# 2alaaa/distributed-llm-scheduler

Hardware: AMD Instinct MI355X
Metric: DAG makespan (ms) + tasks completed under mem cap, GPT-2 DAG at 1/2/4/8 MI355X (lower is better)
Workload: dtype bf16

## Files before the change

csrc/kernels/gemm_glds_impl.h:

```cpp
#pragma once
#include <cstdlib>
#include <type_traits>
#include "common.h"
#include "kernels.h"
#include "gemm_glds_cfgs.h"

#ifndef DLS_STAMP
#define DLS_STAMP(k)
#endif

namespace {

__device__ __forceinline__ int kslice_count(int K, int kslice) { return K / kslice; }

template <int N>
__device__ __forceinline__ void wait_vm() {
  asm volatile("s_waitcnt vmcnt(%0)" ::"n"(N) : "memory");
}
template <int PW, int A>
__device__ __forceinline__ void wait_tiles(int ahead) {
  if constexpr (A == 0) {
    wait_vm<0>();
  } else {
    if (ahead >= A) wait_vm<PW * A>();
    else wait_tiles<PW, A - 1>(ahead);
  }
}
__device__ __forceinline__ void raw_barrier() { asm volatile("s_barrier" ::: "memory"); }

template <int BM_, int BN_, int WM_, int WN_, int STAGES_, int PRIO_ = 0, int BXS_ = 0, int KG_ = 1, int RING_ = 0,
          int OCC_ = 1>
struct Cfg {
  static constexpr int BM = BM_, BN = BN_, WM = WM_, WN = WN_, STAGES = STAGES_, PRIO = PRIO_, BXS = BXS_;
  static constexpr int KG = KG_, RING = RING_, OCC = OCC_;
  static constexpr int BK = 64, CH = 8;
  static constexpr int NW = WM * WN, T = 64 * NW * KG;
  static constexpr int WTM = BM / WM, WTN = BN / WN, FM = WTM / 16, FN = WTN / 16;
  static constexpr bool HALF_FRAGS = FM + FN > 12;
  static constexpr int ROWS = BM + BN, INSTR = ROWS / 8, PW = (INSTR + NW - 1) / NW;
  static constexpr int SUB = ROWS * CH;
  static constexpr int STAGE = SUB * KG;
  static constexpr int SA = STAGES, SB = STAGES + BXS;
  static constexpr int PWA = (BM / 8 + NW - 1) / NW, PWB = (BN / 8 + NW - 1) / NW;
  static constexpr bool EVEN = INSTR % NW == 0, EVEN_A = (BM / 8) % NW == 0, EVEN_B = (BN / 8) % NW == 0;
  static constexpr int A_STAGE = BM * CH, B_STAGE = BN * CH;
  static constexpr int LDS_UNITS = BXS ? SA * A_STAGE + SB * B_STAGE : STAGES * STAGE;
  static_assert(BM % 8 == 0 && BN % 8 == 0, "DMA pieces are 8 rows");
  static_assert(FM >= 1 && FN >= 1, "wave tile too small");
  static_assert(PW * (STAGES - 2) <= 63, "vmcnt range");
  static_assert(!BXS || (SA - 2) * PWA + (SA - 1) * PWB <= 63, "vmcnt range (split rings)");
  static_assert(STAGES >= 2 && STAGES <= 8, "stages");
  static_assert(LDS_UNITS * 16 <= 163840, "LDS budget");
  static_assert(KG == 1 || (BXS == 0 && PRIO == 0), "K groups use the joint ring");
  static_assert(KG == 1 || NW * 64 * FM * FN * 16 <= LDS_UNITS * 16, "K-group reduction must fit the LDS");
  static_assert(!RING || (BM == 256 && BN == 256 && WM == 2 && WN == 4 && STAGES == 2 && KG == 1 && BXS == 0),
                "the ring main loop is written for 256x256 tiles, 8 waves as 2 x 4, 8 x 16 KiB slots");
};

template <int PWA, int PWB, int AM, int BM>
__device__ __forceinline__ void wait_ab_any(int a, int b) {
  if constexpr (AM > 0) {
    if (a < AM) {
      wait_ab_any<PWA, PWB, AM - 1, BM>(a, b);
      return;
    }
  }
  if constexpr (BM > 0) {
    if (b < BM) {
      wait_ab_any<PWA, PWB, AM, BM - 1>(a, b);
      return;
    }
  }
  wait_vm<AM * PWA + BM * PWB>();
}
template <int PWA, int PWB, int A>
__device__ __forceinline__ void wait_ab(int a, int b) {
  if constexpr (A == 0) {
    if (b >= 1) wait_vm<PWB>();
    else wait_vm<0>();
  } else {
    if (a >= A) {
      if (b > A) wait_vm<A * PWA + (A + 1) * PWB>();
      else wait_vm<A * PWA + A * PWB>();
    } else {
      wait_ab<PWA, PWB, A - 1>(a, b);
    }
  }
}

template <class C, bool SKIP = false>
__device__ __forceinline__ void mma_tile(const bf16x8* sA, const bf16x8* sB, int lane, int wm, int wn, bool ln_acc,
                                         f32x4 (&acc)[C::FM][C::FN], float (&st_s)[C::FM], float (&st_q)[C::FM],
                                         int fmv = C::FM) {
  constexpr bool HALVES = C::HALF_FRAGS;
  if constexpr (!HALVES) {
    bf16x8 af[2][C::FM], bw[2][C::FN];
#pragma unroll
    for (int kk = 0; kk < 2; ++kk) {
      const int chunk = kk * 4 + (lane >> 4);
#pragma unroll
      for (int j = 0; j < C::FN; ++j) {
        const int row = wn * C::WTN + j * 16 + (lane & 15);
        bw[kk][j] = sB[row * C::CH + (chunk ^ (row & 7))];
      }
#pragma unroll
      for (int i = 0; i < C::FM; ++i) {
        if (SKIP && i >= fmv) break;
        const int row = wm * C::WTM + i * 16 + (lane & 15);
        af[kk][i] = sA[row * C::CH + (chunk ^ (row & 7))];
      }
    }
    __builtin_amdgcn_sched_barrier(0);
#pragma unroll
    for (int kk = 0; kk < 2; ++kk) {
      if (ln_acc) {
#pragma unroll
        for (int i = 0; i < C::FM; ++i)
#pragma unroll
          for (int e = 0; e < 8; ++e) {
            const float x = bf2f(af[kk][i][e]);
            st_s[i] += x;
            st_q[i] += x * x;
          }
      }
      if constexpr (C::PRIO) __builtin_amdgcn_s_setprio(1);
#pragma unroll
      for (int i = 0; i < C::FM; ++i) {
        if (SKIP && i >= fmv) break;
#pragma unroll
        for (int j = 0; j < C::FN; ++j) acc[i][j] = mfma16x16x32(bw[kk][j], af[kk][i], acc[i][j]);
      }
      if constexpr (C::PRIO) __builtin_amdgcn_s_setprio(0);
    }
  } else {
#pragma unroll
    for (int kk = 0; kk < 2; ++kk) {
      bf16x8 af[C::FM], bw[C::FN];
      const int chunk = kk * 4 + (lane >> 4);
#pragma unroll
      for (int j = 0; j < C::FN; ++j) {
        const int row = wn * C::WTN + j * 16 + (lane & 15);
        bw[j] = sB[row * C::CH + (chunk ^ (row & 7))];
      }
#pragma unroll
      for (int i = 0; i < C::FM; ++i) {
        if (SKIP && i >= fmv) break;
        const int row = wm * C::WTM + i * 16 + (lane & 15);
        af[i] = sA[row * C::CH + (chunk ^ (row & 7))];
      }
      __builtin_amdgcn_sched_barrier(0);
      if (ln_acc) {
#pragma unroll
        for (int i = 0; i < C::FM; ++i)
#pragma unroll
          for (int e = 0; e < 8; ++e) {
            const float x = bf2f(af[i][e]);
            st_s[i] += x;
            st_q[i] += x * x;
          }
      }
      if constexpr (C::PRIO) __builtin_amdgcn_s_setprio(1);
#pragma unroll
      for (int i = 0; i < C::FM; ++i) {
        if (SKIP && i >= fmv) break;
#pragma unroll
        for (int j = 0; j < C::FN; ++j) acc[i][j] = mfma16x16x32(bw[j], af[i], acc[i][j]);
      }
      if constexpr (C::PRIO) __builtin_amdgcn_s_setprio(0);
      __builtin_amdgcn_sched_barrier(0);
    }
  }
}

template <class C, bool GATHER = false, int APOL = 0, int WPOL = 0>
__device__ __forceinline__ void mainloop_joint(bf16x8* smem, const bf16* __restrict__ A, int lda,
                                               const bf16* __restrict__ W, int ldw, int M, int N, int m0, int n0,
                                               int kbeg, int nk, int lane, int wave, int kgrp, int wm, int wn,
                                               bool ln_acc, f32x4 (&acc)[C::FM][C::FN], float (&st_s)[C::FM],
                                               float (&st_q)[C::FM], const int* __restrict__ arows) {
  const bf16* src[C::PW];
  int dst[C::PW];
#pragma unroll
  for (int j = 0; j < C::PW; ++j) {
    const int gi = C::EVEN ? wave * C::PW + j : min(wave * C::PW + j, C::INSTR * C::KG - 1);
    const int sub = gi / C::INSTR, r8 = gi % C::INSTR;
    const int row = 8 * r8 + (lane >> 3);
    const int gch = (lane & 7) ^ (row & 7);
    const int kofs = kbeg + sub * C::BK + gch * 8;
    if (row < C::BM) {
      int gm = min(m0 + row, M - 1);
      if constexpr (GATHER) gm = arows[gm];
      src[j] = A + (size_t)gm * lda + kofs;
    } else {
      const int gn = min(n0 + row - C::BM, N - 1);
      src[j] = W + (size_t)gn * ldw + kofs;
    }
    dst[j] = sub * C::SUB + r8 * 64;
  }
  bool is_a[C::PW];
#pragma unroll
  for (int j = 0; j < C::PW; ++j) {
    const int gi = C::EVEN ? wave * C::PW + j : min(wave * C::PW + j, C::INSTR * C::KG - 1);
    is_a[j] = 8 * (gi % C::INSTR) < C::BM;
  }
  auto issue = [&](int kt) {
    bf16x8* stage = smem + (kt % C::STAGES) * C::STAGE;
#pragma unroll
    for (int j = 0; j < C::PW; ++j) {
      if constexpr (APOL != 0 || WPOL != 0) {
        if (is_a[j])
          __builtin_amdgcn_global_load_lds((const void*)(src[j] + kt * (C::BK * C::KG)),
                                           (__attribute__((address_space(3))) void*)(stage + dst[j]), 16, 0, APOL);
        else
          __builtin_amdgcn_global_load_lds((const void*)(src[j] + kt * (C::BK * C::KG)),
                                           (__attribute__((address_space(3))) void*)(stage + dst[j]), 16, 0, WPOL);
        continue;
      }
      __builtin_amdgcn_global_load_lds((const void*)(src[j] + kt * (C::BK * C::KG)),
                                       (__attribute__((address_space(3))) void*)(stage + dst[j]), 16, 0, 0);
    }
  };
#pragma unroll
  for (int s = 0; s < C::STAGES - 1; ++s)
    if (s < nk) issue(s);
  for (int kt = 0; kt < nk; ++kt) {
    const int ahead = min(C::STAGES - 2, nk - 1 - kt);
    wait_tiles<C::PW, C::STAGES - 2>(ahead);
    raw_barrier();
    if (kt + C::STAGES - 1 < nk) issue(kt + C::STAGES - 1);
    const bf16x8* st = smem + (kt % C::STAGES) * C::STAGE + kgrp * C::SUB;
    mma_tile<C>(st, st + C::BM * C::CH, lane, wm, wn, ln_acc, acc, st_s, st_q);
  }
}

template <class C, int WPOL = 0>
__device__ __forceinline__ void mainloop_ring(bf16x8* smem, const bf16* __restrict__ A, int lda,
                                              const bf16* __restrict__ W, int ldw, int M, int N, int m0, int n0,
                                              int kbeg, int nk, int lane, int wave, int wm, int wn,
                                              f32x4 (&acc)[C::FM][C::FN]) {
  constexpr int SLOT = 128 * 8;
  const bf16* srcA[2][2];
  const bf16* srcB[2][2];
  int dst[2];
#pragma unroll
  for (int j = 0; j < 2; ++j) {
    const int r = 8 * (2 * wave + j) + (lane >> 3);
    const int gch = (lane & 7) ^ (r & 7);
#pragma unroll
    for (int h = 0; h < 2; ++h) {
      srcA[h][j] = A + (size_t)min(m0 + h * 128 + r, M - 1) * lda + kbeg + gch * 8;
      srcB[h][j] = W + (size_t)min(n0 + h * 128 + r, N - 1) * ldw + kbeg + gch * 8;
    }
    dst[j] = (2 * wave + j) * 64;
  }
  auto slot = [&](int t, int hk) { return smem + ((t & 1) * 4 + hk) * SLOT; };
  auto issue = [&](int t, int hk) {
    const bf16* const* src = hk < 2 ? srcA[hk] : srcB[hk - 2];
    bf16x8* st = slot(t, hk);
#pragma unroll
    for (int j = 0; j < 2; ++j) {
      if (hk < 2)
        __builtin_amdgcn_global_load_lds((const void*)(src[j] + t * C::BK),
                                         (__attribute__((address_space(3))) void*)(st + dst[j]), 16, 0, 0);
      else
        __builtin_amdgcn_global_load_lds((const void*)(src[j] + t * C::BK),
                                         (__attribute__((address_space(3))) void*)(st + dst[j]), 16, 0, WPOL);
    }
  };
#pragma unroll
  for (int t = 0; t < 2; ++t)
    if (t < nk) {
      issue(t, 2);
      issue(t, 3);
      issue(t, 0);
      issue(t, 1);
    }
  const int ah = wm;
  const int bh = 2 + (wn >> 1);
  const int brow0 = (wn & 1) * 64;
  bf16x8 af[2][4], bl[2][2], br[2][2];
  for (int t = 0; t < nk; ++t) {
    if (t + 1 < nk) wait_vm<8>();
    else wait_vm<0>();
    raw_barrier();
    const bf16x8* sa = slot(t, ah);
    const bf16x8* sb = slot(t, bh);
#pragma unroll
    for (int kk = 0; kk < 2; ++kk) {
      const int chunk = kk * 4 + (lane >> 4);
#pragma unroll
      for (int i = 0; i < 4; ++i) {
        const int row = i * 16 + (lane & 15);
        af[kk][i] = sa[row * C::CH + (chunk ^ (row & 7))];
      }
#pragma unroll
      for (int j = 0; j < 2; ++j) {
        const int row = brow0 + j * 16 + (lane & 15);
        bl[kk][j] = sb[row * C::CH + (chunk ^ (row & 7))];
      }
    }
    __builtin_amdgcn_sched_barrier(0);
#pragma unroll
    for (int kk = 0; kk < 2; ++kk)
#pragma unroll
      for (int i = 0; i < 4; ++i)
#pragma unroll
        for (int j = 0; j < 2; ++j) acc[i][j] = mfma16x16x32(bl[kk][j], af[kk][i], acc[i][j]);
#pragma unroll
    for (int kk = 0; kk < 2; ++kk) {
      const int chunk = kk * 4 + (lane >> 4);
#pragma unroll
      for (int j = 0; j < 2; ++j) {
        const int row = brow0 + 32 + j * 16 + (lane & 15);
        br[kk][j] = sb[row * C::CH + (chunk ^ (row & 7))];
      }
    }
    __builtin_amdgcn_sched_barrier(0);
#pragma unroll
    for (int kk = 0; kk < 2; ++kk)
#pragma unroll
      for (int i = 0; i < 4; ++i)
#pragma unroll
        for (int j = 0; j < 2; ++j) acc[i][2 + j] = mfma16x16x32(br[kk][j], af[kk][i], acc[i][2 + j]);
    raw_barrier();
    if (t + 2 < nk) {
      issue(t + 2, 2);
      issue(t + 2, 3);
    }
#pragma unroll
    for (int kk = 0; kk < 2; ++kk) {
      const int chunk = kk * 4 + (lane >> 4);
#pragma unroll
      for (int i = 0; i < 4; ++i) {
        const int row = 64 + i * 16 + (lane & 15);
        af[kk][i] = sa[row * C::CH + (chunk ^ (row & 7))];
      }
    }
    __builtin_amdgcn_sched_barrier(0);
#pragma unroll
    for (int kk = 0; kk < 2; ++kk)
#pragma unroll
      for (int i = 0; i < 4; ++i)
#pragma unroll
        for (int j = 0; j < 2; ++j) acc[4 + i][2 + j] = mfma16x16x32(br[kk][j], af[kk][i], acc[4 + i][2 + j]);
    raw_barrier();
    if (t + 2 < nk) {
      issue(t + 2, 0);
      issue(t + 2, 1);
    }
    if constexpr (C::PRIO) __builtin_amdgcn_s_setprio(1);
#pragma unroll
    for (int kk = 0; kk < 2; ++kk)
#pragma unroll
      for (int i = 0; i < 4; ++i)
#pragma unroll
        for (int j = 0; j < 2; ++j) acc[4 + i][j] = mfma16x16x32(bl[kk][j], af[kk][i], acc[4 + i][j]);
    if constexpr (C::PRIO) __builtin_amdgcn_s_setprio(0);
  }
}

constexpr int kPolStream = 2;
constexpr int kPolWT = 16;

template <class C, int WPOL = 0, bool SKIP = false, bool GATHER = false>
__device__ __forceinline__ void mainloop_split(bf16x8* smem, const bf16* __restrict__ A, int lda,
                                               const bf16* __restrict__ W, int ldw, int M, int N, int m0, int n0,
                                               int kbeg, int nk, int lane, int wave, int wm, int wn, bool ln_acc,
                                               f32x4 (&acc)[C::FM][C::FN], float (&st_s)[C::FM],
                                               float (&st_q)[C::FM], int fmv, const int* __restrict__ arows) {
  constexpr int D = C::SB - C::SA;
  static_assert(D >= 1, "split rings: the W ring is deeper than the A ring");
  const bf16* srcA[C::PWA];
  const bf16* srcB[C::PWB];
  uint32_t voffA[C::PWA];
  const auto rsA = __builtin_amdgcn_make_buffer_rsrc((void*)A, 0, 0x7fffffff, 0x00020000);
#pragma unroll
  for (int j = 0; j < C::PWA; ++j) {
    const int row = 8 * (C::EVEN_A ? wave * C::PWA + j : min(wave * C::PWA + j, C::BM / 8 - 1)) + (lane >> 3);
    int gm = min(m0 + row, M - 1);
    if constexpr (GATHER) gm = arows[gm];
    srcA[j] = A + (size_t)gm * lda + kbeg + ((lane & 7) ^ (row & 7)) * 8;
    if constexpr (SKIP)
      voffA[j] = m0 + row < M ? (uint32_t)(((size_t)gm * lda + kbeg + ((lane & 7) ^ (row & 7)) * 8) * 2) : 0x80000000u;
  }
#pragma unroll
  for (int j = 0; j < C::PWB; ++j) {
    const int row = 8 * (C::EVEN_B ? wave * C::PWB + j : min(wave * C::PWB + j, C::BN / 8 - 1)) + (lane >> 3);
    const int gn = min(n0 + row, N - 1);
    srcB[j] = W + (size_t)gn * ldw + kbeg + ((lane & 7) ^ (row & 7)) * 8;
  }
  bf16x8* ringA = smem;
  bf16x8* ringB = smem + C::SA * C::A_STAGE;
  auto issueA = [&](int kt) {
    bf16x8* st = ringA + (kt % C::SA) * C::A_STAGE;
#pragma unroll
    for (int j = 0; j < C::PWA; ++j) {
      auto* dst = (__attribute__((address_space(3))) void*)(st + (C::EVEN_A ? wave * C::PWA + j : min(wave * C::PWA + j, C::BM / 8 - 1)) * 64);
      if constexpr (SKIP)
        __builtin_amdgcn_raw_ptr_buffer_load_lds(rsA, dst, 16, voffA[j] + kt * C::BK * 2, 0, 0, 0);
      else
        __builtin_amdgcn_global_load_lds((const void*)(srcA[j] + kt * C::BK), dst, 16, 0, 0);
    }
  };
  auto issueB = [&](int kt) {
    bf16x8* st = ringB + (kt % C::SB) * C::B_STAGE;
#pragma unroll
    for (int j = 0; j < C::PWB; ++j)
      __builtin_amdgcn_global_load_lds((const void*)(srcB[j] + kt * C::BK),
                                       (__attribute__((address_space(3))) void*)(st + (C::EVEN_B ? wave * C::PWB + j : min(wave * C::PWB + j, C::BN / 8 - 1)) * 64), 16,
                                       0, WPOL);
  };
  constexpr int DA = C::SA - 1;
#pragma unroll
  for (int q = 0; q < D; ++q)
    if (q < nk) issueB(q);
#pragma unroll
  for (int s = 0; s < DA; ++s) {
    if (s < nk) issueA(s);
    if (s + D < nk) issueB(s + D);
  }
  for (int kt = 0; kt < nk; ++kt) {
    const int a = min(DA - 1, nk - 1 - kt);
    const int b = max(0, min(DA, nk - kt - D));
    if constexpr (D == 1) wait_ab<C::PWA, C::PWB, DA - 1>(a, b);
    else wait_ab_any<C::PWA, C::PWB, DA - 1, DA>(a, b);
    raw_barrier();
    if (kt + DA < nk) issueA(kt + DA);
    if (kt + DA + D < nk) issueB(kt + DA + D);
    mma_tile<C, SKIP>(ringA + (kt % C::SA) * C::A_STAGE, ringB + (kt % C::SB) * C::B_STAGE, lane, wm, wn, ln_acc,
                      acc, st_s, st_q, fmv);
  }
}

template <class C, int LN, int WPOL = 0, bool SKIP = false, bool GATHER = false, int APOL = 0, bool PUB = false,
          int SPOL = 0>
__device__ __forceinline__ void glds_tile(bf16x8* smem, const bf16* __restrict__ A, int lda,
                                          const bf16* __restrict__ W, int ldw, bf16* __restrict__ Cp, int ldc,
                                          const bf16* __restrict__ bias, const bf16* __restrict__ R, int ldr,
                                          float* __restrict__ part, int M, int Mmax, int N, int K, int act,
                                          float alpha, int ks, int kslice, int tm, int tn,
                                          const float* __restrict__ ln_colsum, int ln_mode, float ln_eps,
                                          const Epi& ep, const int* __restrict__ arows = nullptr) {
  const RopeArgs& rope = ep.rope;
  const int tid = threadIdx.x, lane = tid & 63, wave = tid >> 6;
  const int kgrp = wave / C::NW, wq = wave % C::NW;
  const int wm = wq / C::WN, wn = wq % C::WN;
  const int m0 = tm * C::BM, n0 = tn * C::BN;
  if (m0 >= M) return;
  DLS_STAMP(0)
  const int kbeg = ks * kslice;
  const int nk = kslice / (C::BK * C::KG);

  f32x4 acc[C::FM][C::FN];
#pragma unroll
  for (int i = 0; i < C::FM; ++i)
#pragma unroll
    for (int j = 0; j < C::FN; ++j) acc[i][j] = f32x4{0.f, 0.f, 0.f, 0.f};
  const bool ln_acc = LN && ln_mode != 0 && wn == 0;
  float st_s[C::FM], st_q[C::FM];
#pragma unroll
  for (int i = 0; i < C::FM; ++i) st_s[i] = st_q[i] = 0.f;
  if constexpr (C::RING && !SKIP && !GATHER)
    mainloop_ring<C, WPOL>(smem, A, lda, W, ldw, M, N, m0, n0, kbeg, nk, lane, wave, wm, wn, acc);
  else if constexpr (C::BXS > 0)
    mainloop_split<C, WPOL, SKIP, GATHER>(smem, A, lda, W, ldw, M, N, m0, n0, kbeg, nk, lane, wave, wm, wn, ln_acc, acc,
                                  st_s, st_q, min(C::FM, max(0, (M - m0 - wm * C::WTM + 15) / 16)), arows);
  else
    mainloop_joint<C, GATHER, APOL, WPOL>(smem, A, lda, W, ldw, M, N, m0, n0, kbeg, nk, lane, wave, kgrp, wm, wn, ln_acc, acc,
                                    st_s, st_q, arows);
  DLS_STAMP(1)
  if constexpr (C::KG > 1) {
    __syncthreads();
    f32x4* red = reinterpret_cast<f32x4*>(smem);
    for (int g2 = 1; g2 < C::KG; ++g2) {
      if (kgrp == g2) {
#pragma unroll
        for (int i = 0; i < C::FM; ++i)
#pragma unroll
          for (int j = 0; j < C::FN; ++j) red[((i * C::FN + j) * C::NW + wq) * 64 + lane] = acc[i][j];
      }
      __syncthreads();
      if (kgrp == 0) {
#pragma unroll
        for (int i = 0; i < C::FM; ++i)
#pragma unroll
          for (int j = 0; j < C::FN; ++j) acc[i][j] += red[((i * C::FN + j) * C::NW + wq) * 64 + lane];
      }
      __syncthreads();
    }
  }

  const int g4 = (lane >> 4) * 4, r16 = lane & 15;
  if (part != nullptr && ep.tile_sem != nullptr) {
    const size_t slab = (size_t)Mmax * N;
    const int tiles_m = (M + C::BM - 1) / C::BM;
    int* sem = ep.tile_sem + tm + tn * tiles_m;
    const auto rsrc = __builtin_amdgcn_make_buffer_rsrc(part, 0, (int)(slab * kslice_count(K, kslice) * 4), 0x00020000);
    if (kgrp == 0) {
#pragma unroll
      for (int i = 0; i < C::FM; ++i) {
        const int row = m0 + wm * C::WTM + i * 16 + r16;
        if (row >= M) continue;
#pragma unroll
        for (int j = 0; j < C::FN; ++j) {
          const int col = n0 + wn * C::WTN + j * 16 + g4;
          if (col >= N) continue;
          const f32x4 v = acc[i][j];
          u32x4 u = {__float_as_uint(v[0]), __float_as_uint(v[1]), __float_as_uint(v[2]), __float_as_uint(v[3])};
          __builtin_amdgcn_raw_buffer_store_b128(u, rsrc, (int)(((size_t)ks * slab + (size_t)row * N + col) * 4), 0,
                                                 16);
        }
      }
    }
    asm volatile("s_waitcnt vmcnt(0)" ::: "memory");
    __syncthreads();
    int* flag = reinterpret_cast<int*>(smem);
    if (threadIdx.x == 0) {
      const int old = __hip_atomic_fetch_add(sem, 1, __ATOMIC_RELAXED, __HIP_MEMORY_SCOPE_AGENT);
      const int last = old == kslice_count(K, kslice) - 1;
      if (last) __hip_atomic_store(sem, 0, __ATOMIC_RELAXED, __HIP_MEMORY_SCOPE_AGENT);
      flag[0] = last;
    }
    __syncthreads();
    const bool last = flag[0] != 0;
    if (!last) return;
    if (kgrp == 0) {
      const int nsl = kslice_count(K, kslice);
      for (int s2 = 0; s2 < nsl; ++s2) {
        if (s2 == ks) continue;
#pragma unroll
        for (int i = 0; i < C::FM; ++i) {
          const int row = min(m0 + wm * C::WTM + i * 16 + r16, M - 1);
#pragma unroll
          for (int j = 0; j < C::FN; ++j) {
            const int col = min(n0 + wn * C::WTN + j * 16 + g4, N - 4);
            const u32x4 u = __builtin_amdgcn_raw_buffer_load_b128(
                rsrc, (int)(((size_t)s2 * slab + (size_t)row * N + col) * 4), 0, 16);
            acc[i][j] += f32x4{__uint_as_float(u[0]), __uint_as_float(u[1]), __uint_as_float(u[2]),
                               __uint_as_float(u[3])};
          }
        }
      }
    }
    part = nullptr;
  }
  float ln_rs[C::FM], ln_mu[C::FM];
  if (ln_mode != 0) {
    if constexpr (LN) {
    float* stats = reinterpret_cast<float*>(smem);
    raw_barrier();
    if (ln_acc) {
#pragma unroll
      for (int i = 0; i < C::FM; ++i) {
        float a = st_s[i], q = st_q[i];
        a += __shfl_xor(a, 16, 64);
        a += __shfl_xor(a, 32, 64);
        q += __shfl_xor(q, 16, 64);
        q += __shfl_xor(q, 32, 64);
        if (lane < 16) {
          const int lr = wm * C::WTM + i * 16 + lane;
          stats[2 * lr] = a;
          stats[2 * lr + 1] = q;
        }
      }
    }
    __syncthreads();
#pragma unroll
    for (int i = 0; i < C::FM; ++i) {
      const int lr = wm * C::WTM + i * 16 + r16;
      const float a = stats[2 * lr], q = stats[2 * lr + 1];
      const float inv_k = 1.0f / (float)K;
      if (ln_mode == 1) {
        const float mu = a * inv_k;
        const float var = fmaxf(q * inv_k - mu * mu, 0.f);
        ln_mu[i] = mu;
        ln_rs[i] = rsqrtf(var + ln_eps);
      } else {
        ln_mu[i] = 0.f;
        ln_rs[i] = rsqrtf(q * inv_k + ln_eps);
      }
    }
      } else {
      const float inv_k = 1.0f / (float)K;
#pragma unroll
      for (int i = 0; i < C::FM; ++i) {
        const int row = min(m0 + wm * C::WTM + i * 16 + r16, M - 1);
        const float a = ep.ext_stats[2 * row], q = ep.ext_stats[2 * row + 1];
        const float mu = ln_mode == 1 ? a * inv_k : 0.f;
        ln_mu[i] = mu;
        ln_rs[i] = rsqrtf(fmaxf(q * inv_k - mu * mu, 0.f) + ln_eps);
      }
    }
  }
  const bool vec_ok = (ldc % 4 == 0) && (!R || ldr % 4 == 0);
  if (part != nullptr) {
    if (kgrp != 0) return;
    float* P = part + (size_t)ks * Mmax * N;
#pragma unroll
    for (int i = 0; i < C::FM; ++i) {
      const int row = m0 + wm * C::WTM + i * 16 + r16;
      if (row >= M) continue;
#pragma unroll
      for (int j = 0; j < C::FN; ++j) {
        const int col = n0 + wn * C::WTN + j * 16 + g4;
        if (N % 4 == 0 && col + 3 < N) {
          const f32x4 v = acc[i][j];
          store16_pol<SPOL>(P, ((size_t)row * N + col) * 4,
                            u32x4{__float_as_uint(v[0]), __float_as_uint(v[1]), __float_as_uint(v[2]),
                                  __float_as_uint(v[3])});
        } else {
#pragma unroll
          for (int e = 0; e < 4; ++e)
            if (col + e < N) P[(size_t)row * N + col + e] = acc[i][j][e];
        }
      }
    }
    return;
  }
  if (act == ACT_SWIGLU) {
    if (kgrp != 0) return;
    const int NO = N / 2;
#pragma unroll
    for (int jj = 0; jj < C::FN / 2; ++jj) {
      const int gcol = n0 + wn * C::WTN + jj * 32 + g4;
      const int ocol = (n0 + wn * C::WTN) / 2 + jj * 16 + g4;
      if (ocol >= NO) continue;
      float bg[4] = {0.f, 0.f, 0.f, 0.f}, bu[4] = {0.f, 0.f, 0.f, 0.f};
      float cg[4] = {0.f, 0.f, 0.f, 0.f}, cu[4] = {0.f, 0.f, 0.f, 0.f};
#pragma unroll
      for (int e = 0; e < 4; ++e) {
        if (bias) {
          bg[e] = bf2f(bias[gcol + e]);
          bu[e] = bf2f(bias[gcol + 16 + e]);
        }
        if (ln_mode != 0) {
          cg[e] = ln_colsum[gcol + e];
          cu[e] = ln_colsum[gcol + 16 + e];
        }
      }
#pragma unroll
      for (int i = 0; i < C::FM; ++i) {
        const int row = m0 + wm * C::WTM + i * 16 + r16;
        if (row >= M) continue;
        bf16x4 o;
#pragma unroll
        for (int e = 0; e < 4; ++e) {
          float g = acc[i][2 * jj][e], u = acc[i][2 * jj + 1][e];
          if (ln_mode != 0) {
            g = ln_rs[i] * (g - ln_mu[i] * cg[e]);
            u = ln_rs[i] * (u - ln_mu[i] * cu[e]);
          } else {
            g *= alpha;
            u *= alpha;
          }
          o[e] = f2bf(silu(g + bg[e]) * (u + bu[e]));
        }
        if (vec_ok && ocol + 3 < NO) {
          store8_pol<SPOL>(Cp, ((size_t)row * ldc + ocol) * 2, *reinterpret_cast<const u32x2*>(&o));
        } else {
#pragma unroll
          for (int e = 0; e < 4; ++e)
            if (ocol + e < NO) Cp[(size_t)row * ldc + ocol + e] = o[e];
        }
      }
    }
    return;
  }
  constexpr int BNC = C::BN / 8;
  constexpr int BNP = BNC <= 8 ? 8 : BNC <= 16 ? 16 : BNC <= 32 ? 32 : 64;
  static_assert(C::BN % 8 == 0 && BNC <= 64, "staged epilogue: BN % 8 == 0, BN <= 512");
  static_assert(C::BM * BNP * 16 <= C::LDS_UNITS * 16, "output tile image must fit the staging LDS");
  static_assert((C::BM * BNP) % 64 == 0 && ((C::BM * BNP) % C::T == 0 || C::BM * BNP < C::T),
                "store pass: every wave makes the same number of passes (shuffles stay wave-uniform)");
  bf16* img = reinterpret_cast<bf16*>(smem);
  __syncthreads();
  auto image_pass = [&](auto act_tag, auto ln_tag, auto rope_tag) {
    constexpr int ACT = decltype(act_tag)::value;
    constexpr bool LNM = decltype(ln_tag)::value, ROPE = decltype(rope_tag)::value;
#pragma unroll
    for (int j = 0; j < C::FN; ++j) {
      if (kgrp != 0) break;
      const int cl = wn * C::WTN + j * 16 + g4;
      const int col = n0 + cl;
      const bool full = col + 3 < N;
      float bv[4] = {0.f, 0.f, 0.f, 0.f};
      float csv[4] = {0.f, 0.f, 0.f, 0.f};
      if (bias) {
#pragma unroll
        for (int e = 0; e < 4; ++e) bv[e] = col + e < N ? bf2f(bias[col + e]) : 0.f;
      }
      if constexpr (LNM) {
        if (full && (N % 4 == 0)) {
          const f32x4 c4 = *reinterpret_cast<const f32x4*>(ln_colsum + col);
#pragma unroll
          for (int e = 0; e < 4; ++e) csv[e] = c4[e];
        } else {
#pragma unroll
          for (int e = 0; e < 4; ++e) csv[e] = col + e < N ? ln_colsum[col + e] : 0.f;
        }
      }
#pragma unroll
      for (int i = 0; i < C::FM; ++i) {
        const int rl = wm * C::WTM + i * 16 + r16;
        float v[4];
        if constexpr (LNM) {
#pragma unroll
          for (int e = 0; e < 4; ++e) v[e] = act_c<ACT>(ln_rs[i] * (acc[i][j][e] - ln_mu[i] * csv[e]) + bv[e]);
        } else {
#pragma unroll
          for (int e = 0; e < 4; ++e) v[e] = act_c<ACT>(alpha * acc[i][j][e] + bv[e]);
        }
        if constexpr (ROPE) rope_pairs<4>(v, m0 + rl, col, rope);
        bf16x4 o;
#pragma unroll
        for (int e = 0; e < 4; ++e) o[e] = f2bf(v[e]);
        *reinterpret_cast<bf16x4*>(img + rl * BNP * 8 + (((cl >> 3) ^ (rl & 7)) << 3) + (cl & 7)) = o;
      }
    }
  };
  using B0 = std::integral_constant<bool, false>;
  using B1 = std::integral_constant<bool, true>;
  auto by_ln = [&](auto act_tag, auto rope_tag) {
    if (ln_mode != 0) image_pass(act_tag, B1{}, rope_tag);
    else image_pass(act_tag, B0{}, rope_tag);
  };
  if (rope.cols) {
    by_ln(std::integral_constant<int, ACT_NONE>{}, B1{});
  } else {
    switch (act) {
      case ACT_GELU_TANH: by_ln(std::integral_constant<int, ACT_GELU_TANH>{}, B0{}); break;
      case ACT_SILU: by_ln(std::integral_constant<int, ACT_SILU>{}, B0{}); break;
      case ACT_RELU: by_ln(std::integral_constant<int, ACT_RELU>{}, B0{}); break;
      default: by_ln(std::integral_constant<int, ACT_NONE>{}, B0{}); break;
    }
  }
  __syncthreads();
  DLS_STAMP(2)
  const bool v16 = ((reinterpret_cast<uintptr_t>(Cp) | ((uintptr_t)ldc * 2)) & 15) == 0 &&
                   (!R || ((reinterpret_cast<uintptr_t>(R) | ((uintptr_t)ldr * 2)) & 15) == 0);
  const bf16x8* img8 = reinterpret_cast<const bf16x8*>(img);
  const int tid_ = threadIdx.x;
#pragma unroll 2
  for (int q = tid_; q < C::BM * BNP; q += C::T) {
    const int rl = q / BNP, cc = q % BNP;
    const int row = m0 + rl, col = n0 + cc * 8;
    bf16x8 o = img8[rl * BNP + (cc ^ (rl & 7))];
    float s1 = 0.f, s2 = 0.f;
    if (cc < BNC && row < M && col < N) {
      if (v16 && col + 8 <= N) {
        if (R) {
          const bf16x8 r8 = *reinterpret_cast<const bf16x8*>(R + (size_t)row * ldr + col);
#pragma unroll
          for (int e = 0; e < 8; ++e) o[e] = f2bf(bf2f(o[e]) + bf2f(r8[e]));
        }
        if constexpr (PUB || SPOL != 0) {
          const auto rs = __builtin_amdgcn_make_buffer_rsrc(Cp, 0, 0x7fffffff, 0x00020000);
          __builtin_amdgcn_raw_buffer_store_b128(*reinterpret_cast<const u32x4*>(&o), rs,
                                                 (int)(((size_t)row * ldc + col) * 2), 0, PUB ? 16 : SPOL);
        } else {
          *reinterpret_cast<bf16x8*>(Cp + (size_t)row * ldc + col) = o;
        }
#pragma unroll
        for (int e = 0; e < 8; ++e) {
          const float y = bf2f(o[e]);
          s1 += y;
          s2 += y * y;
        }
      } else {
#pragma unroll
        for (int e = 0; e < 8; ++e) {
          if (col + e >= N) continue;
          float x = bf2f(o[e]);
          if (R) x += bf2f(R[(size_t)row * ldr + col + e]);
          const bf16 ob = f2bf(x);
          Cp[(size_t)row * ldc + col + e] = ob;
          const float y = bf2f(ob);
          s1 += y;
          s2 += y * y;
        }
      }
    }
    if (ep.stats_out) {
#pragma unroll
      for (int o_ = 1; o_ < BNP; o_ <<= 1) {
        s1 += __shfl_xor(s1, o_, 64);
        s2 += __shfl_xor(s2, o_, 64);
      }
      if (cc == 0 && row < M) {
        atomicAdd(ep.stats_out + 2 * row, s1);
        atomicAdd(ep.stats_out + 2 * row + 1, s2);
      }
    }
  }
  DLS_STAMP(3)
}

template <class C>
struct TallTile {
  using type = void;
};
template <class C>
constexpr int tall_lds_units() {
  if constexpr (std::is_void_v<typename TallTile<C>::type>) return 0;
  else return TallTile<C>::type::LDS_UNITS;
}

template <class C, int LN, int RANGED, int POL = 0>
__global__ __launch_bounds__(C::T, C::OCC) void gemm_glds_kernel(const bf16* __restrict__ A, int lda,
                                                         const bf16* __restrict__ W, int ldw, bf16* __restrict__ Cp,
                                                         int ldc, const bf16* __restrict__ bias,
                                                         const bf16* __restrict__ R, int ldr,
                                                         float* __restrict__ part, int M, int N, int K, int act,
                                                         float alpha, int tiles_m, int tiles_n, int splitk,
                                                         int kslice, const float* __restrict__ ln_colsum,
                                                         int ln_mode, float ln_eps, const int* __restrict__ rows,
                                                         int compact_rows, Epi ep) {
  constexpr int kUnits = RANGED == 3 && tall_lds_units<C>() > C::LDS_UNITS ? tall_lds_units<C>() : C::LDS_UNITS;
  __shared__ bf16x8 smem[kUnits];
  const int ntile = tiles_m * tiles_n;
  if constexpr (RANGED == 2) {
    const int total = ntile * splitk;
    for (int L = blockIdx.x, it = 0; L < total; L += gridDim.x, ++it) {
      if (it) raw_barrier();
      const int ks = L / ntile, tile = L % ntile;
      glds_tile<C, LN>(smem, A, lda, W, ldw, Cp, ldc, bias, R, ldr, part, M, M, N, K, act, alpha, ks, kslice,
                       tile % tiles_m, tile / tiles_m, ln_colsum, (LN || ep.ext_stats) ? ln_mode : 0, ln_eps, ep);
    }
    return;
  }
  if constexpr (RANGED == 3) {
    int g = blockIdx.x / tiles_n, tn = blockIdx.x % tiles_n, t0 = 0, dt = 1;
    if (ep.w_stream & 8) {
      const int L = xcd_remap(blockIdx.x, gridDim.x), ng = gridDim.x / tiles_n;
      tn = L / ng;
      g = L % ng;
    } else if (ep.w_stream & 16) {
      const int pair = (blockIdx.x >> 4) * 8 + (blockIdx.x & 7);
      if (pair >= tiles_m * tiles_n) return;
      g = pair / tiles_n;
      tn = pair % tiles_n;
      t0 = (blockIdx.x >> 3) & 1;
      dt = 2;
    } else if (ep.w_stream & (32 | 64)) {
      const int half = gridDim.x >> 1, second = blockIdx.x >= half, idx = blockIdx.x - second * half;
      t0 = second == ((ep.w_stream & 32) != 0);
      dt = 2;
      g = idx / tiles_n;
      tn = idx % tiles_n;
    }
    if ((ep.w_stream & 128) && !(ep.w_stream & (8 | 16))) {
      const int total = tiles_m * tiles_n, idx = g * tiles_n + tn;
      const int x = idx & 7, j = idx >> 3, q = total >> 3, r = total & 7;
      const int L = x * q + min(x, r) + j;
      g = L / tiles_n;
      tn = L % tiles_n;
    }
    const int r0 = rows[g], cnt = rows[g + 1] - r0;
    const int Mr = compact_rows ? min(cnt, compact_rows) : cnt;
    const bf16* Wg = reinterpret_cast<const bf16*>(ep.grp_w[g]);
    bf16* Cg = ep.grp_c ? reinterpret_cast<bf16*>(ep.grp_c[g]) : Cp + (size_t)r0 * ldc;
    const int* a_rows = reinterpret_cast<const int*>(part);
    const int* ag = a_rows ? a_rows + r0 : nullptr;
    const bf16* Ag = a_rows ? A : A + (size_t)r0 * lda;
    if constexpr (!std::is_void_v<typename TallTile<C>::type>) {
      using T2 = typename TallTile<C>::type;
      constexpr int SPLIT = C::BN / T2::BN;
      static_assert((SPLIT == 1 || SPLIT == 2) && T2::BN * SPLIT == C::BN && T2::BM > C::BM && T2::T == C::T,
                    "a taller tile of the same panel (or of half of it)");
      if ((ep.w_stream & 256) && Mr > C::BM && Mr <= T2::BM) {
        const bool nt = T2::BXS > 0 && (ep.w_stream & 1);
        for (int hh = t0; hh < SPLIT; hh += dt) {
          if (hh != t0) raw_barrier();
          const int tn2 = tn * SPLIT + hh;
          if (a_rows) {
            if (nt)
              glds_tile<T2, 0, kPolStream, true, true>(smem, Ag, lda, Wg, ldw, Cg, ldc, bias, nullptr, 0, nullptr, Mr,
                                                       M, N, K, act, alpha, 0, K, 0, tn2, ln_colsum, 0, ln_eps, ep, ag);
            else
              glds_tile<T2, 0, 0, false, true>(smem, Ag, lda, Wg, ldw, Cg, ldc, bias, nullptr, 0, nullptr, Mr, M, N,
                                               K, act, alpha, 0, K, 0, tn2, ln_colsum, 0, ln_eps, ep, ag);
          } else {
            if (nt)
              glds_tile<T2, 0, kPolStream, true, false>(smem, Ag, lda, Wg, ldw, Cg, ldc, bias, nullptr, 0, nullptr,
                                                        Mr, M, N, K, act, alpha, 0, K, 0, tn2, ln_colsum, 0, ln_eps, ep,
                                                        ag);
            else
              glds_tile<T2, 0, 0, false, false>(smem, Ag, lda, Wg, ldw, Cg, ldc, bias, nullptr, 0, nullptr, Mr, M, N,
                                                K, act, alpha, 0, K, 0, tn2, ln_colsum, 0, ln_eps, ep, ag);
          }
        }
        return;
      }
    }
#define DLS_GROUPED_WALK(GA)                                                                                      \
  for (int t = t0; t * C::BM < Mr; t += dt) {                                                                      \
    if (t != t0) raw_barrier();           \
    if (C::BXS > 0 && (ep.w_stream & 1))                                                                           \
      glds_tile<C, 0, kPolStream, true, GA>(smem, Ag, lda, Wg, ldw, Cg, ldc, bias, nullptr, 0, nullptr, Mr, M, N, K, \
                                            act, alpha, 0, K, t, tn, ln_colsum, 0, ln_eps, ep, ag);                \
    else                                                                                                           \
      glds_tile<C, 0, 0, false, GA>(smem, Ag, lda, Wg, ldw, Cg, ldc, bias, nullptr, 0, nullptr, Mr, M, N, K, act,   \
                                    alpha, 0, K, t, tn, ln_colsum, 0, ln_eps, ep, ag);                             \
  }
    if (a_rows) {
      DLS_GROUPED_WALK(true)
    } else {
      DLS_GROUPED_WALK(false)
    }
#undef DLS_GROUPED_WALK
    return;
  }
  const int bid = xcd_remap(blockIdx.x, ntile * splitk);
  int ks = bid / ntile, tile = bid % ntile;
  int tm = tile % tiles_m, tn = tile / tiles_m;
  if constexpr (!RANGED) {
    if (compact_rows > 0) {
      const int a = compact_rows, b = (ntile >> 3) / a, gm = tiles_m / a;
      const int xcd = blockIdx.x & 7, idx = blockIdx.x >> 3;
      tm = (xcd % gm) * a + idx % a;
      tn = (xcd / gm) * b + idx / a;
      ks = 0;
    }
    glds_tile<C, LN, (POL & 1) ? kPolStream : 0, false, false, 0, false,
              ((POL & 2) ? kPolStream : 0) | ((POL & 4) ? kPolWT : 0)>(
        smem, A, lda, W, ldw, Cp, ldc, bias, R, ldr, part, M, M, N, K, act, alpha, ks, kslice, tm, tn, ln_colsum,
        (LN || ep.ext_stats) ? ln_mode : 0, ln_eps, ep);
    return;
  }
  const int r0 = rows[0], Mr = compact_rows ? min(rows[1] - r0, compact_rows) : rows[1] - r0;
  A += (size_t)r0 * lda;
  if (!compact_rows) Cp += (size_t)r0 * ldc;
  if (R) R += (size_t)r0 * ldr;
  if (part) part += (size_t)r0 * N;
  for (int t = 0; t * C::BM < Mr; ++t) {
    if (t) raw_barrier();
    glds_tile<C, 0>(smem, A, lda, W, ldw, Cp, ldc, bias, R, ldr, part, Mr, M, N, K, act, alpha, ks, kslice, t, tn,
                    ln_colsum, 0, ln_eps, ep);
  }
}

inline int xcd_block(int tiles_m, int tiles_n, size_t a_bytes, size_t w_bytes) {
  static const bool on = [] {
    const char* e = std::getenv("DLS_XCD_BLOCK");
    return e && *e == '1';
  }();
  const int ntile = tiles_m * tiles_n;
  if (!on || ntile % 8 || ntile < 64) return 0;
  const int per = ntile / 8;
  const size_t cur = (size_t)std::min(per, tiles_m) * a_bytes + (size_t)((per + tiles_m - 1) / tiles_m) * w_bytes;
  size_t best = cur;
  int best_a = 0;
  for (int a = 1; a <= per; ++a) {
    if (per % a || tiles_m % a) continue;
    const int b = per / a;
    if (tiles_n % b || (tiles_m / a) * (tiles_n / b) != 8) continue;
    const size_t c = (size_t)a * a_bytes + (size_t)b * w_bytes;
    if (c < best) {
      best = c;
      best_a = a;
    }
  }
  return best * 10 < cur * 9 ? best_a : 0;
}

template <class C, int LN>
int persistent_grid() {
  static int g = 0;
  if (!g) {
    int dev = 0, cus = 256, per = 1;
    (void)hipGetDevice(&dev);
    (void)hipDeviceGetAttribute(&cus, hipDeviceAttributeMultiprocessorCount, dev);
    (void)hipOccupancyMaxActiveBlocksPerMultiprocessor(&per, gemm_glds_kernel<C, LN, 2>, C::T, 0);
    g = cus * (per > 0 ? per : 1);
  }
  return g;
}

template <class C>
bool launch(const GemmArgs& a, int splitk, float* ws, hipStream_t s, const float* ln_colsum, int ln_mode,
            float ln_eps, const int* rows, bool persist) {
  static const int fixup_max = [] {
    const char* e = std::getenv("DLS_FIXUP_MAX_KB");
    return (e && *e ? std::atoi(e) : 64) * 1024;
  }();
  const bool fixup = splitk > 1 && !rows && (splitk - 1) * C::BM * C::BN * 4 <= fixup_max;
  int spol = a.stream_pol & 7;
  if ((size_t)a.M * a.ldc * 2 >= (1ull << 31) || (size_t)a.M * a.N * 4 * splitk >= (1ull << 31)) spol &= 1;
  const Epi ep{a.rope, a.stats_out, a.ext_stats, fixup ? a.tile_sem : nullptr, nullptr, nullptr, spol & 4};
  const int crows = rows ? a.compact_rows
                         : (!persist && splitk == 1 ? xcd_block((a.M + C::BM - 1) / C::BM, (a.N + C::BN - 1) / C::BN,
                                                                (size_t)C::BM * a.K * 2, (size_t)C::BN * a.K * 2)
                                                    : 0);
  static_assert(2 * C::BM * sizeof(float) <= C::LDS_UNITS * 16, "LN stats must fit the staging LDS");
  const int tiles_m = rows ? 1 : (a.M + C::BM - 1) / C::BM, tiles_n = (a.N + C::BN - 1) / C::BN;
  const int kslice = a.K / splitk;
  const int total = tiles_m * tiles_n * splitk;
  dim3 grid(total), block(C::T);
#define DLS_K(LN_, RG_, ...)                                                                                      \
  hipLaunchKernelGGL((gemm_glds_kernel<C, LN_, RG_, ##__VA_ARGS__>), grid, block, 0, s, (const bf16*)a.A, a.lda, (const bf16*)a.W, \
                     a.ldw, (bf16*)a.C, a.ldc, (const bf16*)a.bias, (const bf16*)a.R, a.ldr, ws, a.M, a.N, a.K, a.act, \
                     a.alpha, tiles_m, tiles_n, splitk, kslice, ln_colsum, ln_mode, ln_eps, rows, crows, ep)
  const bool ln_in = ln_mode != 0 && !a.ext_stats;
  if (rows) DLS_K(0, 1);
  else if (persist) {
    if (ln_in) {
      if constexpr (C::BM * C::BN <= 256 * 128 && C::KG == 1) {
        grid = dim3(std::min(total, persistent_grid<C, 1>()));
        DLS_K(1, 2);
      }
    } else {
      grid = dim3(std::min(total, persistent_grid<C, 0>()));
      DLS_K(0, 2);
    }
  } else if (ln_in) {
    if constexpr (C::BM * C::BN <= 256 * 128 && C::KG == 1) DLS_K(1, 0);
  } else {
    const int pol = spol;
    switch (pol) {
      case 1: DLS_K(0, 0, 1); break;
      case 2: DLS_K(0, 0, 2); break;
      case 3: DLS_K(0, 0, 3); break;
      case 4: DLS_K(0, 0, 4); break;
      case 5: DLS_K(0, 0, 5); break;
      default: DLS_K(0, 0);
    }
  }
#undef DLS_K
  if (splitk > 1 && !ep.tile_sem) return glds_reduce(a, splitk, ws, s, ln_colsum, ln_mode, ln_eps, rows, ep);
  return false;
}

using C0 = Cfg<256, 128, 4, 2, 3>;
using C1 = Cfg<128, 128, 2, 2, 3>;
using C2 = Cfg<128, 64, 2, 2, 4>;
using C3 = Cfg<64, 64, 2, 2, 4>;
using C4 = Cfg<64, 128, 2, 2, 4>;
using C5 = Cfg<64, 64, 2, 2, 8>;
using C6 = Cfg<128, 64, 2, 2, 6>;
using C7 = Cfg<128, 128, 2, 2, 4>;
using C8 = Cfg<256, 256, 2, 4, 2>;
using C9 = Cfg<256, 256, 2, 4, 2, 1>;
using C10 = Cfg<256, 128, 4, 2, 3, 1>;
using C11 = Cfg<128, 128, 2, 2, 4, 1>;
using C12 = Cfg<256, 256, 2, 4, 2, 0, 1>;
using C13 = Cfg<256, 256, 2, 4, 2, 1, 1>;
using C14 = Cfg<256, 128, 4, 2, 3, 0, 1>;
using C15 = Cfg<128, 128, 2, 2, 3, 0, 1>;
using C16 = Cfg<64, 64, 2, 2, 3, 0, 0, 2>;
using C17 = Cfg<64, 64, 2, 2, 2, 0, 0, 2>;
using C18 = Cfg<128, 64, 2, 2, 2, 0, 0, 2>;
using C19 = Cfg<64, 128, 2, 2, 2, 0, 0, 2>;
using C20 = Cfg<64, 64, 2, 2, 2, 0, 0, 4>;
using C21 = Cfg<64, 64, 1, 2, 2, 0, 0, 4>;
using C22 = Cfg<64, 96, 2, 2, 4>;
using C23 = Cfg<32, 144, 2, 1, 4>;
using C24 = Cfg<32, 48, 2, 1, 4>;
using C25 = Cfg<64, 96, 2, 2, 3, 0, 0, 2>;
using C26 = Cfg<32, 144, 2, 1, 3, 0, 0, 2>;
using C27 = Cfg<32, 48, 2, 1, 4, 0, 0, 2>;
using C28 = Cfg<128, 128, 2, 2, 2, 0, 0, 2>;
using C29 = Cfg<192, 128, 2, 2, 3>;
using C30 = Cfg<192, 128, 2, 2, 2, 0, 0, 2>;
using C31 = Cfg<192, 128, 2, 2, 2, 0, 1>;
using C32 = Cfg<192, 128, 2, 2, 3, 0, 1>;
using C33 = Cfg<192, 128, 4, 2, 3, 0, 1>;
using C34 = Cfg<256, 256, 2, 4, 2, 0, 0, 1, 1>;
using C35 = Cfg<256, 256, 2, 4, 2, 1, 0, 1, 1>;
using C36 = Cfg<256, 224, 4, 2, 2, 0, 1>;
using C37 = Cfg<256, 224, 8, 1, 2, 0, 1>;
using C38 = Cfg<128, 96, 4, 2, 4>;
using C39 = Cfg<128, 96, 2, 2, 2, 0, 0, 2>;
using C40 = Cfg<128, 64, 2, 2, 3, 0, 0, 2>;
using C41 = Cfg<192, 128, 4, 2, 3, 0, 2>;
using C42 = Cfg<256, 144, 8, 1, 3>;
using C43 = Cfg<256, 192, 4, 2, 2, 0, 1>;
using C44 = Cfg<160, 256, 2, 4, 2, 0, 1>;
using C45 = Cfg<32, 48, 2, 1, 3, 0, 0, 4>;
using C46 = Cfg<128, 128, 2, 2, 2, 0, 0, 1, 0, 2>;
using C47 = Cfg<128, 128, 2, 2, 2, 0, 1, 1, 0, 2>;

template <>
struct TallTile<C44> {
  using type = Cfg<224, 256, 2, 4, 2, 0, 1>;
};
template <>
struct TallTile<C33> {
  using type = C14;
};

template <class C>
void grouped(const GemmArgs& a, int n_groups, const int* offsets, const unsigned long long* w_ptrs,
             const unsigned long long* c_ptrs, hipStream_t s, const int* a_rows) {
  static const int w_stream = [] {
    const char* e = std::getenv("DLS_EXPERT_NT");
    return e && e[0] == '0' ? 0 : 1;
  }();
  const char* pe = std::getenv("DLS_EXPERT_PAIRS");
  const int pairs = pe && *pe ? std::atoi(pe) : 2;
  const int pair = a.grouped_shared ? 0 : pairs;
  const char* xe = std::getenv("DLS_EXPERT_XCD");
  const bool xcd = xe && *xe == '1' && !a.grouped_shared && pair != 1;
  const char* te = std::getenv("DLS_EXPERT_TALL");
  const bool tall = !(te && *te == '0') && !a.grouped_shared;
  const Epi ep{a.rope, nullptr, nullptr, nullptr, w_ptrs, c_ptrs,
               (a.grouped_shared ? 8 : ((size_t)a.M * a.lda * 2 < (1ull << 31) ? w_stream : 0)) |
                   (pair == 1 ? 16 : pair == 2 ? 32 : pair == 3 ? 64 : 0) | (xcd ? 128 : 0) | (tall ? 256 : 0)};
  const int tiles_n = (a.N + C::BN - 1) / C::BN;
  const int blocks = pair == 1 ? (n_groups * tiles_n + 7) / 8 * 16 : pair >= 2 ? 2 * n_groups * tiles_n
                                                                               : n_groups * tiles_n;
  hipLaunchKernelGGL((gemm_glds_kernel<C, 0, 3>), dim3(blocks), dim3(C::T), 0, s, (const bf16*)a.A, a.lda,
                     nullptr, a.ldw, (bf16*)a.C, a.ldc, nullptr, nullptr, 0,
                     const_cast<float*>(reinterpret_cast<const float*>(a_rows)), a.M, a.N, a.K, a.act, a.alpha,
                     n_groups, tiles_n, 1, a.K, nullptr, 0, 1e-5f, offsets, a.compact_rows, ep);
}

}

#define DLS_GLDS_DEFINE(ID)                                                                                     \
  bool glds_launch_cfg##ID(const GemmArgs& a, int splitk, float* ws, hipStream_t s, const float* ln_colsum,     \
                           int ln_mode, float ln_eps, const int* rows, bool persist) {                          \
    return launch<C##ID>(a, splitk, ws, s, ln_colsum, ln_mode, ln_eps, rows, persist);                          \
  }                                                                                                             \
  void glds_grouped_cfg##ID(const GemmArgs& a, int n_groups, const int* offsets, const unsigned long long* w_ptrs, \
                            const unsigned long long* c_ptrs, hipStream_t s, const int* a_rows) {               \
    grouped<C##ID>(a, n_groups, offsets, w_ptrs, c_ptrs, s, a_rows);                                            \
  }
```

Measured before the change: 0.6093.

## Prefetch epilogue operands before K-group reduction and use LDS-only barriers

For small-fragment configs, the GEMM epilogue now issues buffer loads for bias, LN column sums, external row stats and the residual tile into registers before the K-group reduction. The values are consumed later, so global-load latency overlaps with the reduction and image pass. Epilogue barriers wait only on LDS counters instead of the full __syncthreads, so the in-flight global loads do not stall them. For KG>2 the reduction becomes a single-shot layout using (KG-1) LDS slabs. The cost is higher register pressure and more complex per-pass residual selection.

After: 0.5719, median of 6. 1.07x faster.

```diff
diff --git a/csrc/kernels/gemm_glds_impl.h b/csrc/kernels/gemm_glds_impl.h
--- a/csrc/kernels/gemm_glds_impl.h
+++ b/csrc/kernels/gemm_glds_impl.h
@@ -27,6 +27,15 @@
   }
 }
 __device__ __forceinline__ void raw_barrier() { asm volatile("s_barrier" ::: "memory"); }
+template <class T>
+__device__ __forceinline__ void consume_from_here(T& x) {
+  asm volatile("" : "+v"(x));
+}
+template <bool WAIT_LDS_ONLY>
+__device__ __forceinline__ void epi_barrier() {
+  if constexpr (WAIT_LDS_ONLY) asm volatile("s_waitcnt lgkmcnt(0)\n\ts_barrier" ::: "memory");
+  else __syncthreads();
+}
 
 template <int BM_, int BN_, int WM_, int WN_, int STAGES_, int PRIO_ = 0, int BXS_ = 0, int KG_ = 1, int RING_ = 0,
           int OCC_ = 1>
@@ -52,7 +61,8 @@
   static_assert(STAGES >= 2 && STAGES <= 8, "stages");
   static_assert(LDS_UNITS * 16 <= 163840, "LDS budget");
   static_assert(KG == 1 || (BXS == 0 && PRIO == 0), "K groups use the joint ring");
-  static_assert(KG == 1 || NW * 64 * FM * FN * 16 <= LDS_UNITS * 16, "K-group reduction must fit the LDS");
+  static_assert(KG == 1 || (KG - 1) * NW * 64 * FM * FN * 16 <= LDS_UNITS * 16, "K-group reduction must fit the LDS");
+  static constexpr bool EPI_BATCH = FM * FN <= 4;
   static_assert(!RING || (BM == 256 && BN == 256 && WM == 2 && WN == 4 && STAGES == 2 && KG == 1 && BXS == 0),
                 "the ring main loop is written for 256x256 tiles, 8 waves as 2 x 4, 8 x 16 KiB slots");
 };
@@ -469,8 +479,93 @@
     mainloop_joint<C, GATHER, APOL, WPOL>(smem, A, lda, W, ldw, M, N, m0, n0, kbeg, nk, lane, wave, kgrp, wm, wn, ln_acc, acc,
                                     st_s, st_q, arows);
   DLS_STAMP(1)
-  if constexpr (C::KG > 1) {
-    __syncthreads();
+  const int g4 = (lane >> 4) * 4, r16 = lane & 15;
+  constexpr int BNC = C::BN / 8;
+  constexpr int BNP = BNC <= 8 ? 8 : BNC <= 16 ? 16 : BNC <= 32 ? 32 : 64;
+  constexpr int NPASS = (C::BM * BNP + C::T - 1) / C::T;
+  const bool pre_bvec = ((reinterpret_cast<uintptr_t>(bias) & 7) | (N & 3)) == 0;
+  const bool pre_cvec = ((reinterpret_cast<uintptr_t>(ln_colsum) & 15) | (N & 3)) == 0;
+  const bool pre_res = C::EPI_BATCH && R != nullptr && N >= 8 && ((size_t)(M + C::BM) * ldr * 2 < (1ull << 31)) &&
+                       ((reinterpret_cast<uintptr_t>(Cp) | ((uintptr_t)ldc * 2) | reinterpret_cast<uintptr_t>(R) |
+                         ((uintptr_t)ldr * 2)) & 15) == 0;
+  u32x2 pre_bv[C::FN];
+  uint32_t pre_bs[C::FN][4];
+  u32x4 pre_cs[C::FN];
+  u32x2 pre_st[C::FM];
+  u32x4 pre_r[NPASS];
+  auto request_operands = [&]() {
+    constexpr int kRaw = 0x00020000;
+    if (kgrp == 0) {
+      if (ln_mode != 0 && !LN) {
+        const auto rs = __builtin_amdgcn_make_buffer_rsrc(const_cast<float*>(ep.ext_stats), 0, M * 8, kRaw);
+        const int vo = (m0 + wm * C::WTM + r16) * 8;
+#pragma unroll
+        for (int i = 0; i < C::FM; ++i) pre_st[i] = __builtin_amdgcn_raw_buffer_load_b64(rs, vo + i * 128, 0, 0);
+      }
+      const int c0 = n0 + wn * C::WTN + g4;
+      if (bias) {
+        if (pre_bvec) {
+          const auto rs = __builtin_amdgcn_make_buffer_rsrc(const_cast<bf16*>(bias), 0, N * 2, kRaw);
+#pragma unroll
+          for (int j = 0; j < C::FN; ++j) pre_bv[j] = __builtin_amdgcn_raw_buffer_load_b64(rs, c0 * 2 + j * 32, 0, 0);
+        } else {
+          const unsigned short* b16 = reinterpret_cast<const unsigned short*>(bias);
+#pragma unroll
+          for (int j = 0; j < C::FN; ++j)
+#pragma unroll
+            for (int e = 0; e < 4; ++e) pre_bs[j][e] = b16[min(c0 + j * 16 + e, N - 1)];
+        }
+      }
+      if (ln_mode != 0) {
+        if (pre_cvec) {
+          const auto rs = __builtin_amdgcn_make_buffer_rsrc(const_cast<float*>(ln_colsum), 0, N * 4, kRaw);
+#pragma unroll
+          for (int j = 0; j < C::FN; ++j) pre_cs[j] = __builtin_amdgcn_raw_buffer_load_b128(rs, c0 * 4 + j * 64, 0, 0);
+        } else {
+          const uint32_t* c32 = reinterpret_cast<const uint32_t*>(ln_colsum);
+#pragma unroll
+          for (int j = 0; j < C::FN; ++j)
+#pragma unroll
+            for (int e = 0; e < 4; ++e) pre_cs[j][e] = c32[min(c0 + j * 16 + e, N - 1)];
+        }
+      }
+    }
+    if (pre_res) {
+      const auto rs = __builtin_amdgcn_make_buffer_rsrc(const_cast<bf16*>(R), 0, (int)(((size_t)(M - 1) * ldr + N) * 2), kRaw);
+#pragma unroll
+      for (int p = 0; p < NPASS; ++p) {
+        const int q = tid + p * C::T;
+        if (q < C::BM * BNP)
+          pre_r[p] = __builtin_amdgcn_raw_buffer_load_b128(rs, ((m0 + q / BNP) * ldr + n0 + (q % BNP) * 8) * 2, 0, 0);
+      }
+    }
+  };
+  if constexpr (C::EPI_BATCH) {
+    if (part == nullptr && act != ACT_SWIGLU) request_operands();
+  }
+  if constexpr (C::KG > 2) {
+    constexpr int REG = C::NW * C::FM * C::FN * 64;
+    epi_barrier<C::EPI_BATCH>();
+    f32x4* red = reinterpret_cast<f32x4*>(smem);
+    if (kgrp != 0) {
+#pragma unroll
+      for (int i = 0; i < C::FM; ++i)
+#pragma unroll
+        for (int j = 0; j < C::FN; ++j)
+          red[(kgrp - 1) * REG + ((i * C::FN + j) * C::NW + wq) * 64 + lane] = acc[i][j];
+    }
+    epi_barrier<C::EPI_BATCH>();
+    if (kgrp == 0) {
+#pragma unroll
+      for (int g2 = 1; g2 < C::KG; ++g2)
+#pragma unroll
+        for (int i = 0; i < C::FM; ++i)
+#pragma unroll
+          for (int j = 0; j < C::FN; ++j)
+            acc[i][j] += red[(g2 - 1) * REG + ((i * C::FN + j) * C::NW + wq) * 64 + lane];
+    }
+  } else if constexpr (C::KG > 1) {
+    epi_barrier<C::EPI_BATCH>();
     f32x4* red = reinterpret_cast<f32x4*>(smem);
     for (int g2 = 1; g2 < C::KG; ++g2) {
       if (kgrp == g2) {
@@ -479,18 +574,18 @@
 #pragma unroll
           for (int j = 0; j < C::FN; ++j) red[((i * C::FN + j) * C::NW + wq) * 64 + lane] = acc[i][j];
       }
-      __syncthreads();
+      epi_barrier<C::EPI_BATCH>();
       if (kgrp == 0) {
 #pragma unroll
         for (int i = 0; i < C::FM; ++i)
 #pragma unroll
           for (int j = 0; j < C::FN; ++j) acc[i][j] += red[((i * C::FN + j) * C::NW + wq) * 64 + lane];
       }
-      __syncthreads();
-    }
-  }
-
-  const int g4 = (lane >> 4) * 4, r16 = lane & 15;
+      epi_barrier<C::EPI_BATCH>();
+    }
+  }
+
+  DLS_STAMP(7)
   if (part != nullptr && ep.tile_sem != nullptr) {
     const size_t slab = (size_t)Mmax * N;
     const int tiles_m = (M + C::BM - 1) / C::BM;
@@ -524,6 +619,9 @@
     __syncthreads();
     const bool last = flag[0] != 0;
     if (!last) return;
+    if constexpr (C::EPI_BATCH) {
+      if (act != ACT_SWIGLU) request_operands();
+    }
     if (kgrp == 0) {
       const int nsl = kslice_count(K, kslice);
       for (int s2 = 0; s2 < nsl; ++s2) {
@@ -584,8 +682,19 @@
       const float inv_k = 1.0f / (float)K;
 #pragma unroll
       for (int i = 0; i < C::FM; ++i) {
-        const int row = min(m0 + wm * C::WTM + i * 16 + r16, M - 1);
-        const float a = ep.ext_stats[2 * row], q = ep.ext_stats[2 * row + 1];
+        float a, q;
+        if (C::EPI_BATCH && act != ACT_SWIGLU) {
+          a = q = 0.f;
+          if (kgrp == 0) {
+            consume_from_here(pre_st[i]);
+            a = __uint_as_float(pre_st[i][0]);
+            q = __uint_as_float(pre_st[i][1]);
+          }
+        } else {
+          const int row = min(m0 + wm * C::WTM + i * 16 + r16, M - 1);
+          a = ep.ext_stats[2 * row];
+          q = ep.ext_stats[2 * row + 1];
+        }
         const float mu = ln_mode == 1 ? a * inv_k : 0.f;
         ln_mu[i] = mu;
         ln_rs[i] = rsqrtf(fmaxf(q * inv_k - mu * mu, 0.f) + ln_eps);
@@ -666,14 +775,12 @@
     }
     return;
   }
-  constexpr int BNC = C::BN / 8;
-  constexpr int BNP = BNC <= 8 ? 8 : BNC <= 16 ? 16 : BNC <= 32 ? 32 : 64;
   static_assert(C::BN % 8 == 0 && BNC <= 64, "staged epilogue: BN % 8 == 0, BN <= 512");
   static_assert(C::BM * BNP * 16 <= C::LDS_UNITS * 16, "output tile image must fit the staging LDS");
   static_assert((C::BM * BNP) % 64 == 0 && ((C::BM * BNP) % C::T == 0 || C::BM * BNP < C::T),
                 "store pass: every wave makes the same number of passes (shuffles stay wave-uniform)");
   bf16* img = reinterpret_cast<bf16*>(smem);
-  __syncthreads();
+  epi_barrier<C::EPI_BATCH>();
   auto image_pass = [&](auto act_tag, auto ln_tag, auto rope_tag) {
     constexpr int ACT = decltype(act_tag)::value;
     constexpr bool LNM = decltype(ln_tag)::value, ROPE = decltype(rope_tag)::value;
@@ -685,6 +792,35 @@
       const bool full = col + 3 < N;
       float bv[4] = {0.f, 0.f, 0.f, 0.f};
       float csv[4] = {0.f, 0.f, 0.f, 0.f};
+      if constexpr (C::EPI_BATCH) {
+        if (bias) {
+#pragma unroll
+          for (int e = 0; e < 4; ++e) bv[e] = 0.f;
+          uint32_t w[4];
+          if (pre_bvec) {
+            consume_from_here(pre_bv[j]);
+            const uint32_t p0 = pre_bv[j][0], p1 = pre_bv[j][1];
+            w[0] = p0 << 16;
+            w[1] = p0 & 0xffff0000u;
+            w[2] = p1 << 16;
+            w[3] = p1 & 0xffff0000u;
+          } else {
+#pragma unroll
+            for (int e = 0; e < 4; ++e) {
+              consume_from_here(pre_bs[j][e]);
+              w[e] = pre_bs[j][e] << 16;
+            }
+          }
+#pragma unroll
+          for (int e = 0; e < 4; ++e) bv[e] = col + e < N ? __uint_as_float(w[e]) : 0.f;
+        }
+        if constexpr (LNM) {
+          consume_from_here(pre_cs[j]);
+#pragma unroll
+          for (int e = 0; e < 4; ++e) csv[e] = col + e < N ? __uint_as_float(pre_cs[j][e]) : 0.f;
+        }
+        (void)full;
+      } else {
       if (bias) {
 #pragma unroll
         for (int e = 0; e < 4; ++e) bv[e] = col + e < N ? bf2f(bias[col + e]) : 0.f;
@@ -698,6 +834,7 @@
 #pragma unroll
           for (int e = 0; e < 4; ++e) csv[e] = col + e < N ? ln_colsum[col + e] : 0.f;
         }
+      }
       }
 #pragma unroll
       for (int i = 0; i < C::FM; ++i) {
@@ -734,10 +871,17 @@
       default: by_ln(std::integral_constant<int, ACT_NONE>{}, B0{}); break;
     }
   }
-  __syncthreads();
+  epi_barrier<C::EPI_BATCH>();
   DLS_STAMP(2)
   const bool v16 = ((reinterpret_cast<uintptr_t>(Cp) | ((uintptr_t)ldc * 2)) & 15) == 0 &&
                    (!R || ((reinterpret_cast<uintptr_t>(R) | ((uintptr_t)ldr * 2)) & 15) == 0);
+  if constexpr (C::EPI_BATCH) {
+    if (pre_res) {
+#pragma unroll
+      for (int p = 0; p < NPASS; ++p)
+        if (tid + p * C::T < C::BM * BNP) consume_from_here(pre_r[p]);
+    }
+  }
   const bf16x8* img8 = reinterpret_cast<const bf16x8*>(img);
   const int tid_ = threadIdx.x;
 #pragma unroll 2
@@ -749,7 +893,16 @@
     if (cc < BNC && row < M && col < N) {
       if (v16 && col + 8 <= N) {
         if (R) {
-          const bf16x8 r8 = *reinterpret_cast<const bf16x8*>(R + (size_t)row * ldr + col);
+          bf16x8 r8;
+          if constexpr (C::EPI_BATCH) {
+            u32x4 rp = pre_r[0];
+#pragma unroll
+            for (int p = 1; p < NPASS; ++p) rp = q / C::T == p ? pre_r[p] : rp;
+            r8 = pre_res ? *reinterpret_cast<const bf16x8*>(&rp)
+                         : *reinterpret_cast<const bf16x8*>(R + (size_t)row * ldr + col);
+          } else {
+            r8 = *reinterpret_cast<const bf16x8*>(R + (size_t)row * ldr + col);
+          }
 #pragma unroll
           for (int e = 0; e < 8; ++e) o[e] = f2bf(bf2f(o[e]) + bf2f(r8[e]));
         }
```
